# chansoopark98/Deep-Visual-SLAM

Hardware: AMD Instinct MI355X
Metric: VO training-step frames/sec (3-frame 640x480 snippets) (higher is better)
Workload: dtype f32; 1 GPU; configs[2]/[3]: full 4-scale photometric+smoothness loss, batch 12 per GPU, ResNet-18; per_gpu_batch=12, global_batch=12, num_scales=4, image=640x480, parallelism=dp1, streams=depth | pose | 2x weight-gradient, optimizer=fused Adam pass at lr 0: every step computes from the seeded weights, gpu_max_hw_queues=4

## Files before the change

deep-visual-slam_amd/csrc/loss_chain.hip:

```cpp
#include "common.h"

namespace {

constexpr int TW = 64, TH = 16, NT = 256, PX = 4;
constexpr int FH = TH + 2, FW = TW + 2;
constexpr int BH = TH + 4, BW = TW + 4;
constexpr int ACC_W = TW / 2 + 4, ACC_H = TH / 2 + 4;
constexpr int NPART = 16;
constexpr int NDP = 12;
constexpr float C1 = 0.0001f, C2 = 0.0009f;
constexpr float K9 = 1.0f / 9.0f;
#ifndef FWD_WAVES
#define FWD_WAVES 3
#endif
#ifndef BWD_WAVES
#define BWD_WAVES 2
#endif
#ifndef CHAIN_DBG
#define CHAIN_DBG 0
#endif
#ifndef BWD_NT
#define BWD_NT 256
#endif
constexpr int FIELD_ROWS = 6, FIELD_THREADS = FW * (FH / FIELD_ROWS);
static_assert(FH % FIELD_ROWS == 0 && FIELD_THREADS <= NT, "field strips must tile the 1-px-halo tile");
static_assert(ACC_H * ACC_W <= 3 * FH * FW, "sAcc aliases sF");

struct ChainParams {
    dvs_chain_cfg cfg;
    dvs_chain_fwd_io io;
    int tiles_x, tiles_y;
};

struct CamMats {
    float iK[9];
    float P[12];
};

__device__ __forceinline__ float frcp(float x) { return __builtin_amdgcn_rcpf(x); }

__device__ __forceinline__ int reflect_idx(int i, int n) {
    i = i < 0 ? -i : i;
    i = i >= n ? 2 * n - 2 - i : i;
    return min(max(i, 0), n - 1);
}

__device__ __forceinline__ void load_cam(const ChainParams& p, int b, int f, CamMats& m) {
    const float* K = p.io.K + b * 16;
    const float* T = p.io.T[f] + b * 16;
    const float* iK = p.io.inv_K + b * 16;
#pragma unroll
    for (int i = 0; i < 3; ++i) {
#pragma unroll
        for (int j = 0; j < 4; ++j) {
            float acc = K[i * 4 + 0] * T[0 * 4 + j];
            acc = fmaf(K[i * 4 + 1], T[1 * 4 + j], acc);
            acc = fmaf(K[i * 4 + 2], T[2 * 4 + j], acc);
            acc = fmaf(K[i * 4 + 3], T[3 * 4 + j], acc);
            m.P[i * 4 + j] = acc;
        }
#pragma unroll
        for (int j = 0; j < 3; ++j) m.iK[i * 3 + j] = iK[i * 4 + j];
    }
}

__device__ __forceinline__ float disp_up_at(const float* __restrict__ d, int hs, int ws, bool same_res, int W,
                                            int X, int Y, float ry, float rx) {
    if (same_res) return d[Y * W + X];
    float sy = fmaxf(ry * (Y + 0.5f) - 0.5f, 0.f);
    float sx = fmaxf(rx * (X + 0.5f) - 0.5f, 0.f);
    int y0 = min((int)sy, hs - 1), x0 = min((int)sx, ws - 1);
    int y1 = y0 + (y0 < hs - 1), x1 = x0 + (x0 < ws - 1);
    float ly = sy - y0, lx = sx - x0;
    float v00 = d[y0 * ws + x0], v01 = d[y0 * ws + x1];
    float v10 = d[y1 * ws + x0], v11 = d[y1 * ws + x1];
    return (1.f - ly) * ((1.f - lx) * v00 + lx * v01) + ly * ((1.f - lx) * v10 + lx * v11);
}

struct Geo {
    float min_disp, disp_range;
    float inv_wm1, inv_hm1, wm1, hm1;
    int H, W;
};

struct Warp {
    float depth, c0, c1, c2;
    float rden, u, v;
    float gx, gy;
    float mx, my;
    int x0, y0;
    float tx, ty;
    bool in_x1, in_y1;
};

__device__ __forceinline__ void pixel_ray(const float* __restrict__ iK, int X, int Y, float& c0, float& c1, float& c2) {
    float fx = (float)X, fy = (float)Y;
    c0 = fmaf(iK[1], fy, iK[0] * fx) + iK[2];
    c1 = fmaf(iK[4], fy, iK[3] * fx) + iK[5];
    c2 = fmaf(iK[7], fy, iK[6] * fx) + iK[8];
}

__device__ __forceinline__ void warp_project(const float* __restrict__ P, const Geo& g, float depth, float c0, float c1,
                                             float c2, Warp& w) {
    w.depth = depth;
    w.c0 = c0;
    w.c1 = c1;
    w.c2 = c2;
    float X3 = depth * c0, Y3 = depth * c1, Z3 = depth * c2;
    float p0 = fmaf(P[2], Z3, fmaf(P[1], Y3, P[0] * X3)) + P[3];
    float p1 = fmaf(P[6], Z3, fmaf(P[5], Y3, P[4] * X3)) + P[7];
    float p2 = fmaf(P[10], Z3, fmaf(P[9], Y3, P[8] * X3)) + P[11];
    w.rden = frcp(p2 + 1e-7f);
    w.u = p0 * w.rden;
    w.v = p1 * w.rden;
// ... 113 lines not shown
                                            float outb[PX]) {
    float ssa[PX] = {0.f, 0.f, 0.f, 0.f}, ssb[PX] = {0.f, 0.f, 0.f, 0.f};
    float l1a[PX] = {0.f, 0.f, 0.f, 0.f}, l1b[PX] = {0.f, 0.f, 0.f, 0.f};
#pragma unroll 1
    for (int c = 0; c < 3; ++c) {
        const int o = c * PLANE + ly0 * LD + lx;
        const float* xa = sXa + o;
        const float* xb = sXb + o;
        const float* y = sT + o;
        float ry[PX + 2], ryy[PX + 2], ax[PX + 2], axx[PX + 2], axy[PX + 2], bx[PX + 2], bxx[PX + 2], bxy[PX + 2];
#pragma unroll
        for (int j = 0; j < PX + 2; ++j) {
            const float y0 = y[j * LD], y1 = y[j * LD + 1], y2 = y[j * LD + 2];
            const float a0 = xa[j * LD], a1 = xa[j * LD + 1], a2 = xa[j * LD + 2];
            const float b0 = xb[j * LD], b1 = xb[j * LD + 1], b2 = xb[j * LD + 2];
            ry[j] = y0 + y1 + y2;
            ryy[j] = fmaf(y2, y2, fmaf(y1, y1, y0 * y0));
            ax[j] = a0 + a1 + a2;
            axx[j] = fmaf(a2, a2, fmaf(a1, a1, a0 * a0));
            axy[j] = fmaf(a2, y2, fmaf(a1, y1, a0 * y0));
            bx[j] = b0 + b1 + b2;
            bxx[j] = fmaf(b2, b2, fmaf(b1, b1, b0 * b0));
            bxy[j] = fmaf(b2, y2, fmaf(b1, y1, b0 * y0));
            if (j >= 1 && j <= PX) {
                l1a[j - 1] += fabsf(y1 - a1);
                l1b[j - 1] += fabsf(y1 - b1);
            }
        }
#pragma unroll
        for (int k = 0; k < PX; ++k) {
            const float muy = (ry[k] + ry[k + 1] + ry[k + 2]) * K9;
            const float sigy = (ryy[k] + ryy[k + 1] + ryy[k + 2]) * K9 - muy * muy;
            const float my2 = fmaf(muy, muy, C1), sy2 = sigy + C2;
            {
                const float mux = (ax[k] + ax[k + 1] + ax[k + 2]) * K9;
                const float sigx = (axx[k] + axx[k + 1] + axx[k + 2]) * K9 - mux * mux;
                const float sigxy = (axy[k] + axy[k + 1] + axy[k + 2]) * K9 - mux * muy;
                const float n = (2.f * mux * muy + C1) * (2.f * sigxy + C2);
                const float d = fmaf(mux, mux, my2) * (sigx + sy2);
                ssa[k] += fminf(fmaxf((1.f - n * frcp(d)) * 0.5f, 0.f), 1.f);
            }
            {
                const float mux = (bx[k] + bx[k + 1] + bx[k + 2]) * K9;
                const float sigx = (bxx[k] + bxx[k + 1] + bxx[k + 2]) * K9 - mux * mux;
                const float sigxy = (bxy[k] + bxy[k + 1] + bxy[k + 2]) * K9 - mux * muy;
                const float n = (2.f * mux * muy + C1) * (2.f * sigxy + C2);
                const float d = fmaf(mux, mux, my2) * (sigx + sy2);
                ssb[k] += fminf(fmaxf((1.f - n * frcp(d)) * 0.5f, 0.f), 1.f);
            }
        }
    }
#pragma unroll
    for (int k = 0; k < PX; ++k) {
        outa[k] = ssim_ratio * (ssa[k] * (1.f / 3.f)) + (1.f - ssim_ratio) * (l1a[k] * (1.f / 3.f));
        outb[k] = ssim_ratio * (ssb[k] * (1.f / 3.f)) + (1.f - ssim_ratio) * (l1b[k] * (1.f / 3.f));
    }
}

__device__ __forceinline__ void philox4x32(uint32_t c0, uint32_t c1, uint32_t c2, uint32_t c3, uint32_t k0,
                                           uint32_t k1, uint32_t out[4]) {
#pragma unroll
    for (int r = 0; r < 10; ++r) {
        uint32_t hi0 = __umulhi(0xD2511F53u, c0), lo0 = 0xD2511F53u * c0;
        uint32_t hi1 = __umulhi(0xCD9E8D57u, c2), lo1 = 0xCD9E8D57u * c2;
        uint32_t n0 = hi1 ^ c1 ^ k0, n1 = lo1, n2 = hi0 ^ c3 ^ k1, n3 = lo0;
        c0 = n0; c1 = n1; c2 = n2; c3 = n3;
        k0 += 0x9E3779B9u;
        k1 += 0xBB67AE85u;
    }
    out[0] = c0; out[1] = c1; out[2] = c2; out[3] = c3;
}

__device__ __forceinline__ void box_muller(uint32_t a, uint32_t b, float& n0, float& n1) {
    float u1 = ((float)a + 0.5f) * 2.3283064365386963e-10f;
    float u2 = ((float)b + 0.5f) * 2.3283064365386963e-10f;
    float r = sqrtf(-2.f * __logf(u1));
    float s, c;
    __sincosf(6.283185307179586f * u2, &s, &c);
    n0 = r * c;
    n1 = r * s;
}

__device__ __forceinline__ float uni(float v) { return __builtin_bit_cast(float, __builtin_amdgcn_readfirstlane(__builtin_bit_cast(int, v))); }

__device__ __forceinline__ Geo make_geo(const dvs_chain_cfg& c) {
    Geo g;
    g.min_disp = uni(1.0f / c.max_depth);
    g.disp_range = uni(1.0f / c.min_depth - 1.0f / c.max_depth);
    g.wm1 = uni((float)(c.W - 1));
    g.hm1 = uni((float)(c.H - 1));
    g.inv_wm1 = uni(1.0f / g.wm1);
    g.inv_hm1 = uni(1.0f / g.hm1);
    g.H = c.H;
    g.W = c.W;
    return g;
}

template <int PLANE>
__device__ __forceinline__ float edge_weight(const float* __restrict__ sT, int o0, int o1) {
    float gi = fabsf(sT[o0] - sT[o1]) + fabsf(sT[PLANE + o0] - sT[PLANE + o1]) +
               fabsf(sT[2 * PLANE + o0] - sT[2 * PLANE + o1]);
    return __expf(-gi * (1.f / 3.f));
}

constexpr int CAM_STRIDE = 36;
__host__ __device__ __forceinline__ size_t stats_floats(int B, int S) {
    return ((size_t)B * S * 4 + (size_t)B * CAM_STRIDE + 3) / 4 * 4;
}
__device__ __forceinline__ const float* cam_table(const ChainParams& p, int b) {
    return p.io.stats + (size_t)p.cfg.B * p.cfg.num_scales * 4 + (size_t)b * CAM_STRIDE;
}
__device__ __forceinline__ const f4* packed_source(const ChainParams& p, int f, int b) {
    const f4* base = reinterpret_cast<const f4*>(p.io.stats + stats_floats(p.cfg.B, p.cfg.num_scales));
    return base + ((size_t)f * p.cfg.B + b) * ((size_t)p.cfg.H * p.cfg.W);
}

__global__ __launch_bounds__(NT) void chain_pack_kernel(ChainParams p) {
    const int HW = p.cfg.H * p.cfg.W;
    const size_t n = (size_t)2 * p.cfg.B * HW;
    f4* out = reinterpret_cast<f4*>(p.io.stats + stats_floats(p.cfg.B, p.cfg.num_scales));
    for (size_t i = (size_t)blockIdx.x * NT + threadIdx.x; i < n; i += (size_t)gridDim.x * NT) {
        const int pix = (int)(i % HW);
        const size_t fb = i / HW;
        const int b = (int)(fb % p.cfg.B), f = (int)(fb / p.cfg.B);
        const float* src = p.io.source[f] + (size_t)b * 3 * HW + pix;
        out[i] = f4{src[0], src[HW], src[2 * HW], 0.f};
    }
}

__global__ void chain_cam_kernel(ChainParams p) {
    const int b = blockIdx.x, t = threadIdx.x;
    float* out = p.io.stats + (size_t)p.cfg.B * p.cfg.num_scales * 4 + (size_t)b * CAM_STRIDE;
    if (t < 12) {
        const float* iK = p.io.inv_K + b * 16;
        out[t] = (t < 9) ? iK[(t / 3) * 4 + (t % 3)] : 0.f;
    } else if (t < 36) {
        const int f = (t - 12) / 12, e = (t - 12) % 12, i = e / 4, j = e % 4;
        const float* K = p.io.K + b * 16;
        const float* T = p.io.T[f] + b * 16;
        float acc = K[i * 4 + 0] * T[0 * 4 + j];
        acc = fmaf(K[i * 4 + 1], T[1 * 4 + j], acc);
        acc = fmaf(K[i * 4 + 2], T[2 * 4 + j], acc);
        acc = fmaf(K[i * 4 + 3], T[3 * 4 + j], acc);
        out[t] = acc;
    }
}


__global__ __launch_bounds__(NT, FWD_WAVES) void chain_fwd_kernel(ChainParams p) {
    __shared__ float sT[3 * FH * FW];
    __shared__ float sX[2][3 * FH * FW];
    __shared__ float sD[FH * FW];
    __shared__ uint32_t sH[FH * FW];
    __shared__ float sRed[NT / 64][NPART];

    const dvs_chain_cfg& c = p.cfg;
    const int H = c.H, W = c.W, HW = H * W, S = c.num_scales;
    const int b = blockIdx.z, X0 = blockIdx.x * TW, Y0 = blockIdx.y * TH;
    const int tid = threadIdx.x, tx = tid & 63, ty = tid >> 6;
    const Geo geo = make_geo(c);
    constexpr int PL = FH * FW;
    const int X = X0 + tx, Yb = Y0 + PX * ty;

    const float* tgt = p.io.target + (size_t)b * 3 * HW;
    const float* src0 = p.io.source[0] + (size_t)b * 3 * HW;
    const float* src1 = p.io.source[1] + (size_t)b * 3 * HW;
// ... 110 lines not shown
                float i0 = ident[0][k] + n0 * 0.00001f, i1 = ident[1][k] + n1 * 0.00001f;
                best = i0;
                idx = 0;
                if (i1 < best) { best = i1; idx = 1; }
                if (rp[0][k] < best) { best = rp[0][k]; idx = 2; }
            }
            if (rp[1][k] < best) { best = rp[1][k]; idx = 3; }
            a_min += best;
            selbits[k] |= idx << (2 * s);

            int o = (PX * ty + k + 1) * FW + tx + 1;
            float d0 = sD[o];
            a_disp += d0;
            if (X < W - 1) a_gx += fabsf(d0 - sD[o + 1]) * edge_weight<PL>(sT, o, o + 1);
            if (Y < H - 1) a_gy += fabsf(d0 - sD[o + FW]) * edge_weight<PL>(sT, o, o + FW);
        }
        a_min = dvs::wave_sum(a_min);
        a_disp = dvs::wave_sum(a_disp);
        a_gx = dvs::wave_sum(a_gx);
        a_gy = dvs::wave_sum(a_gy);
        if (lane == 0) {
            sRed[wave][s * 4 + 0] = a_min;
            sRed[wave][s * 4 + 1] = a_disp;
            sRed[wave][s * 4 + 2] = a_gx;
            sRed[wave][s * 4 + 3] = a_gy;
        }
        __syncthreads();
    }

#pragma unroll
    for (int k = 0; k < PX; ++k) {
        int Y = Yb + k;
        if (X < W && Y < H) p.io.sel[(size_t)b * HW + (size_t)Y * W + X] = (uint8_t)selbits[k];
    }

    if (tid < NPART) {
        float v = sRed[0][tid] + sRed[1][tid] + sRed[2][tid] + sRed[3][tid];
        int tile = blockIdx.y * p.tiles_x + blockIdx.x;
        p.io.partials[((size_t)b * p.tiles_x * p.tiles_y + tile) * NPART + tid] = v;
    }
}

__global__ __launch_bounds__(NT) void chain_fwd_reduce_kernel(ChainParams p) {
    __shared__ float sRed[NT / 64][NPART];
    const int b = blockIdx.x, ntiles = p.tiles_x * p.tiles_y, tid = threadIdx.x;
    const int col = tid & 15;
    float v = 0.f;
    for (int r = tid >> 4; r < ntiles; r += NT / 16) v += p.io.partials[((size_t)b * ntiles + r) * NPART + col];
    v += __shfl_xor(v, 16, 64);
    v += __shfl_xor(v, 32, 64);
    if ((tid & 63) < 16) sRed[tid >> 6][col] = v;
    __syncthreads();
    if (tid < NPART) {
        float t = sRed[0][tid] + sRed[1][tid] + sRed[2][tid] + sRed[3][tid];
        int s = tid >> 2, j = tid & 3;
        if (s < p.cfg.num_scales) p.io.stats[((size_t)b * p.cfg.num_scales + s) * 4 + j] = t;
    }
}

__global__ void chain_fwd_losses_kernel(ChainParams p) {
    const dvs_chain_cfg& c = p.cfg;
    int s = threadIdx.x;
    if (s >= c.num_scales) return;
    float minsum = 0.f, gx = 0.f, gy = 0.f;
    float hw = (float)c.H * (float)c.W;
    for (int b = 0; b < c.B; ++b) {
        const float* st = p.io.stats + ((size_t)b * c.num_scales + s) * 4;
        float mean = fmaxf(st[1] / hw, 0.001f) + 1e-7f;
        minsum += st[0];
        gx += st[2] / mean;
        gy += st[3] / mean;
    }
    float nx = (float)c.B * (float)c.H * (float)(c.W - 1), ny = (float)c.B * (float)(c.H - 1) * (float)c.W;
    float smooth = gx / nx + gy / ny;
    p.io.losses[s] = minsum / ((float)c.B * hw) + c.smoothness_ratio * smooth / (float)(1 << s);
}

struct BwdParams {
    dvs_chain_bwd_io g;
};

__device__ __forceinline__ float sgn(float v) { return (v > 0.f) ? 1.f : ((v < 0.f) ? -1.f : 0.f); }

template <int NTB, int PXB>
__global__ __launch_bounds__(NTB, NTB == 512 ? 4 : BWD_WAVES) void chain_bwd_kernel(ChainParams p, BwdParams q) {
    static_assert((NTB / 64) * PXB == TH, "waves x rows per lane = tile height");
    constexpr int NWV = NTB / 64;
    constexpr int RING = BH * BW - TH * TW;
    constexpr int FR = NTB == 512 ? 3 : FIELD_ROWS, FT = FW * (FH / FR);
    static_assert(FH % FR == 0 && FT <= NTB, "field strips must tile the 1-px-halo tile");
    __shared__ float sT[3 * BH * BW];
    __shared__ float sX[3 * BH * BW];
    __shared__ float sD[BH * BW];
    __shared__ float sF[3 * FH * FW];
    __shared__ uint8_t sSel[FH * FW];
    __shared__ uint32_t sH[BH * BW];
    __shared__ float sRed[NTB / 64][NDP];
    float* sAcc = sF;

    const dvs_chain_cfg& c = p.cfg;
    const int H = c.H, W = c.W, HW = H * W, S = c.num_scales;
    const int b = blockIdx.z, X0 = blockIdx.x * TW, Y0 = blockIdx.y * TH;
    const int tid0 = threadIdx.x;
    const int wave = tid0 >> 6, lane = tid0 & 63;
    const Geo geo = make_geo(c);
    constexpr int PLB = BH * BW, PLF = FH * FW;
    const int tile = blockIdx.y * p.tiles_x + blockIdx.x, ntiles = p.tiles_x * p.tiles_y;
    int tid = tid0;

    const float* tgt = p.io.target + (size_t)b * 3 * HW;
    for (int i = tid; i < PLB; i += NTB) {
        int hy = i / BW, hx = i - hy * BW;
        int gx = reflect_idx(X0 - 2 + hx, W), gy = reflect_idx(Y0 - 2 + hy, H);
        sH[i] = (uint32_t)gx | ((uint32_t)gy << 16);
#pragma unroll
        for (int ch = 0; ch < 3; ++ch) sT[ch * PLB + i] = tgt[ch * HW + gy * W + gx];
    }
    const float* cam = cam_table(p, b);
    for (int i = tid; i < PLF; i += NTB) {
        int hy = i / FW, hx = i - hy * FW;
        int px = X0 - 1 + hx, py = Y0 - 1 + hy;
        bool in = px >= 0 && px < W && py >= 0 && py < H;
        sSel[i] = in ? p.io.sel[(size_t)b * HW + (size_t)py * W + px] : (uint8_t)0;
    }
    __syncthreads();

    const float w_pix = uni(1.0f / ((float)c.B * (float)HW));
    const float cx = uni(1.0f / ((float)c.B * (float)H * (float)(W - 1)));
    const float cy = uni(1.0f / ((float)c.B * (float)(H - 1) * (float)W));
    const int s_lo = (q.g.scale_end > q.g.scale_begin) ? q.g.scale_begin : 0;
    const int s_hi = (q.g.scale_end > q.g.scale_begin) ? min(q.g.scale_end, S) : S;
#pragma unroll 1
    for (int s = s_lo; s < s_hi; ++s) {
        asm volatile("" : "+v"(tid));
        const int tx = tid & 63, ty = tid >> 6;
        const int X = X0 + tx, Yb = Y0 + PXB * ty;
        const float wxm = (X == 1) ? 2.f : 1.f, wxp = (X == W - 2) ? 2.f : 1.f;
        const int fcol = tid % FW, frow0 = (tid / FW) * FR;
        const bool field_thread = tid < FT;
        const int fpx = X0 - 1 + fcol;
        const int hs = c.hs[s], ws = c.ws[s];
        const bool same_res = (hs == H && ws == W);
        const float* dsp = p.io.disp[s] + (size_t)b * hs * ws;
        const float ry = uni((float)hs / (float)H), rx = uni((float)ws / (float)W);
        const float gl = q.g.d_losses[s];
        const float w_ssim = uni(gl * w_pix * c.ssim_ratio * (1.f / 3.f) * (-0.5f) * K9);
        const float w_l1 = uni(gl * w_pix * (1.f - c.ssim_ratio) * (1.f / 3.f));
        float gd[PXB];
#pragma unroll
        for (int k = 0; k < PXB; ++k) gd[k] = 0.f;

#pragma unroll 1
        for (int f = 0; f < 2; ++f) {
            const float* P = cam + 12 + 12 * f;
            const f4* src4 = packed_source(p, f, b);
            const uint32_t want = 2u + (uint32_t)f;
            auto stage = [&](int i, float (*keep)[2]) __attribute__((always_inline)) {
                const uint32_t h = sH[i];
                const int gx = (int)(h & 0xffffu), gy = (int)(h >> 16);
                float du;
                if (f == 0) {
                    du = disp_up_at(dsp, hs, ws, same_res, W, gx, gy, ry, rx);
                    sD[i] = du;
                } else {
                    du = sD[i];
                }
                float c0, c1, c2;
                pixel_ray(cam, gx, gy, c0, c1, c2);
                Warp w;
                warp_project(P, geo, frcp(geo.min_disp + geo.disp_range * du), c0, c1, c2, w);
                f4 nw, ne, sw, se;
                if (CHAIN_DBG & 1) nw = ne = sw = se = f4{w.u, w.v, w.gx, w.gy};
                else gather_rgba(src4, W, w, nw, ne, sw, se);
                const f4 c4 = bilerp4(w, nw, ne, sw, se);
#pragma unroll
                for (int ch = 0; ch < 3; ++ch) sX[ch * PLB + i] = c4[ch];
                if (keep) {
                    const f4 ddx = ((ne - nw) * (1.f - w.ty) + (se - sw) * w.ty) * (w.mx * w.rden);
                    const f4 ddy = ((sw - nw) * (1.f - w.tx) + (se - ne) * w.tx) * (w.my * w.rden);
#pragma unroll
                    for (int ch = 0; ch < 3; ++ch) {
                        keep[ch][0] = ddx[ch];
                        keep[ch][1] = ddy[ch];
                    }
                }
            };
            float tapd[PXB][3][2];
#pragma unroll
            for (int k = 0; k < PXB; ++k) stage((PXB * ty + k + 2) * BW + tx + 2, tapd[k]);
            for (int j = tid; j < RING; j += NTB) {
                int i;
                if (j < 2 * BW) i = j;
                else if (j < 4 * BW) i = (BH - 4) * BW + j;
                else {
                    const int r = j - 4 * BW, c = r & 3;
                    i = (2 + (r >> 2)) * BW + (c < 2 ? c : BW - 4 + c);
                }
                stage(i, nullptr);
            }
            __syncthreads();

            float dcol[PXB][3];
#pragma unroll 1
            for (int ch = 0; ch < 3; ++ch) {
                if (field_thread && !(CHAIN_DBG & 2)) {
                    const float* xw = sX + ch * PLB + frow0 * BW + fcol;
                    const float* yw = sT + ch * PLB + frow0 * BW + fcol;
                    RowSums r0 = row_sums(xw, yw), r1 = row_sums(xw + BW, yw + BW);
#pragma unroll
                    for (int j = 0; j < FR; ++j) {
                        RowSums r2 = row_sums(xw + (j + 2) * BW, yw + (j + 2) * BW);
                        int hy = frow0 + j, i = hy * FW + fcol, py = Y0 - 1 + hy;
                        float fa = 0.f, fb = 0.f, fc = 0.f;
                        bool in = fpx >= 0 && fpx < W && py >= 0 && py < H;
                        if (in && ((sSel[i] >> (2 * s)) & 3u) == want) {
                            Stats st = stats_of(r0, r1, r2);
                            float n1 = 2.f * st.mux * st.muy + C1, n2 = 2.f * st.sigxy + C2;
                            float d1 = st.mux * st.mux + st.muy * st.muy + C1, d2 = st.sigx + st.sigy + C2;
                            float rd1 = frcp(d1), rd2 = frcp(d2), rd = rd1 * rd2;
                            float R = n1 * n2 * rd, v = (1.f - R) * 0.5f;
                            if (v >= 0.f && v <= 1.f) {
                                float dR_dmux = 2.f * st.muy * n2 * rd - R * 2.f * st.mux * rd1;
                                float dR_dsx = -R * rd2;
                                float dR_dsxy = 2.f * n1 * rd;
                                fa = w_ssim * (dR_dmux - 2.f * st.mux * dR_dsx - st.muy * dR_dsxy);
                                fb = w_ssim * 2.f * dR_dsx;
                                fc = w_ssim * dR_dsxy;
                            }
                        }
                        sF[0 * PLF + i] = fa;
                        sF[1 * PLF + i] = fb;
                        sF[2 * PLF + i] = fc;
                        r0 = r1;
                        r1 = r2;
                    }
                }
                __syncthreads();
                if (CHAIN_DBG & 4) {
#pragma unroll
                    for (int k = 0; k < PXB; ++k) dcol[k][ch] = sX[ch * PLB + (PXB * ty + k + 2) * BW + tx + 2];
                } else {
                    float ha[PXB + 2], hb[PXB + 2], hc[PXB + 2];
#pragma unroll
                    for (int j = 0; j < PXB + 2; ++j) {
                        int o = (PXB * ty + j) * FW + tx;
                        ha[j] = wxm * sF[o] + sF[o + 1] + wxp * sF[o + 2];
                        hb[j] = wxm * sF[PLF + o] + sF[PLF + o + 1] + wxp * sF[PLF + o + 2];
                        hc[j] = wxm * sF[2 * PLF + o] + sF[2 * PLF + o + 1] + wxp * sF[2 * PLF + o + 2];
                    }
#pragma unroll
                    for (int k = 0; k < PXB; ++k) {
                        int Y = Yb + k;
                        float wym = (Y == 1) ? 2.f : 1.f, wyp = (Y == H - 2) ? 2.f : 1.f;
                        float Sa = wym * ha[k] + ha[k + 1] + wyp * ha[k + 2];
                        float Sb = wym * hb[k] + hb[k + 1] + wyp * hb[k + 2];
                        float Sc = wym * hc[k] + hc[k + 1] + wyp * hc[k + 2];
                        int o2 = (PXB * ty + k + 2) * BW + tx + 2;
                        float xq = sX[ch * PLB + o2], yq = sT[ch * PLB + o2];
                        float g = Sa + Sb * xq + Sc * yq;
                        if (((sSel[(PXB * ty + k + 1) * FW + tx + 1] >> (2 * s)) & 3u) == want) g += w_l1 * sgn(xq - yq);
                        dcol[k][ch] = g;
                    }
                }
                __syncthreads();
            }

            float dP[NDP];
#pragma unroll
            for (int j = 0; j < NDP; ++j) dP[j] = 0.f;
#pragma unroll
            for (int k = 0; k < PXB; ++k) {
                int Y = Yb + k;
                if (X >= W || Y >= H) continue;
                if (CHAIN_DBG & 8) {
                    dP[k] += dcol[k][0] + dcol[k][1] + dcol[k][2];
                    continue;
                }
                float du = sD[(PXB * ty + k + 2) * BW + tx + 2];
                float c0, c1, c2;
                pixel_ray(cam, X, Y, c0, c1, c2);
                Warp w;
                warp_project(P, geo, frcp(geo.min_disp + geo.disp_range * du), c0, c1, c2, w);
                float dp0 = 0.f, dp1 = 0.f;
#pragma unroll
                for (int ch = 0; ch < 3; ++ch) {
                    dp0 += dcol[k][ch] * tapd[k][ch][0];
                    dp1 += dcol[k][ch] * tapd[k][ch][1];
                }
                float dp2 = -(dp0 * w.u + dp1 * w.v);
                float X3 = w.depth * w.c0, Y3 = w.depth * w.c1, Z3 = w.depth * w.c2;
                dP[0] += dp0 * X3; dP[1] += dp0 * Y3; dP[2] += dp0 * Z3; dP[3] += dp0;
                dP[4] += dp1 * X3; dP[5] += dp1 * Y3; dP[6] += dp1 * Z3; dP[7] += dp1;
                dP[8] += dp2 * X3; dP[9] += dp2 * Y3; dP[10] += dp2 * Z3; dP[11] += dp2;
                float dc0 = P[0] * dp0 + P[4] * dp1 + P[8] * dp2;
                float dc1 = P[1] * dp0 + P[5] * dp1 + P[9] * dp2;
                float dc2 = P[2] * dp0 + P[6] * dp1 + P[10] * dp2;
                float d_depth = dc0 * w.c0 + dc1 * w.c1 + dc2 * w.c2;
                gd[k] += d_depth * (-w.depth * w.depth * geo.disp_range);
            }
#pragma unroll
            for (int j = 0; j < NDP; ++j) {
                float v = (CHAIN_DBG & 16) ? dP[j] : dvs::wave_sum_lane63(dP[j]);
                if (lane == 63) sRed[wave][j] = v;
            }
            __syncthreads();
            if (tid < NDP) {
                float v = 0.f;
#pragma unroll
                for (int wv = 0; wv < NWV; ++wv) v += sRed[wv][tid];
                q.g.bwd_partials[((((size_t)b * ntiles + tile) * S + s) * 2 + f) * NDP + tid] = v;
            }
            __syncthreads();
        }

        {
            const float* st = p.io.stats + ((size_t)b * S + s) * 4;
            float hw = (float)HW;
            float mean_raw = st[1] / hw;
            float mean = fmaxf(mean_raw, 0.001f) + 1e-7f;
            float gs = gl * c.smoothness_ratio / (float)(1 << s);
            float k_grad = gs / mean;
            float k_mean = (mean_raw >= 0.001f) ? -gs * (cx * st[2] + cy * st[3]) / (mean * mean) / hw : 0.f;
#pragma unroll
            for (int k = 0; k < PXB; ++k) {
                int Y = Yb + k;
                if (X >= W || Y >= H) continue;
                int o = (PXB * ty + k + 2) * BW + tx + 2;
                float d0 = sD[o];
                float g = 0.f;
                if (X < W - 1) g += cx * sgn(d0 - sD[o + 1]) * edge_weight<PLB>(sT, o, o + 1);
                if (X > 0) g -= cx * sgn(sD[o - 1] - d0) * edge_weight<PLB>(sT, o - 1, o);
                if (Y < H - 1) g += cy * sgn(d0 - sD[o + BW]) * edge_weight<PLB>(sT, o, o + BW);
                if (Y > 0) g -= cy * sgn(sD[o - BW] - d0) * edge_weight<PLB>(sT, o - BW, o);
                gd[k] += k_grad * g + k_mean;
            }
        }

        float* dd = q.g.d_disp[s] + (size_t)b * hs * ws;
        if (same_res) {
#pragma unroll
            for (int k = 0; k < PXB; ++k) {
                int Y = Yb + k;
                if (X < W && Y < H) dd[Y * W + X] = gd[k];
            }
        } else {
            for (int i = tid; i < ACC_H * ACC_W; i += NTB) sAcc[i] = 0.f;
            int ox = (int)fmaxf(rx * (X0 + 0.5f) - 0.5f, 0.f), oy = (int)fmaxf(ry * (Y0 + 0.5f) - 0.5f, 0.f);
            __syncthreads();
#pragma unroll
            for (int k = 0; k < PXB; ++k) {
                int Y = Yb + k;
                if (X >= W || Y >= H) continue;
                float sy = fmaxf(ry * (Y + 0.5f) - 0.5f, 0.f), sx = fmaxf(rx * (X + 0.5f) - 0.5f, 0.f);
                int y0 = min((int)sy, hs - 1), x0 = min((int)sx, ws - 1);
                int y1 = y0 + (y0 < hs - 1), x1 = x0 + (x0 < ws - 1);
                float ly = sy - y0, lx = sx - x0;
                float g = gd[k];
                atomicAdd(&sAcc[(y0 - oy) * ACC_W + (x0 - ox)], g * (1.f - ly) * (1.f - lx));
                atomicAdd(&sAcc[(y0 - oy) * ACC_W + (x1 - ox)], g * (1.f - ly) * lx);
                atomicAdd(&sAcc[(y1 - oy) * ACC_W + (x0 - ox)], g * ly * (1.f - lx));
                atomicAdd(&sAcc[(y1 - oy) * ACC_W + (x1 - ox)], g * ly * lx);
            }
            __syncthreads();
            for (int i = tid; i < ACC_H * ACC_W; i += NTB) {
                int ay = i / ACC_W, ax = i - ay * ACC_W;
                float v = sAcc[i];
                int yy = oy + ay, xx = ox + ax;
                if (v != 0.f && yy < hs && xx < ws) atomicAdd(&dd[yy * ws + xx], v);
            }
        }
        __syncthreads();
    }
}

__global__ __launch_bounds__(NT) void chain_bwd_reduce_kernel(ChainParams p, BwdParams q) {
    __shared__ float sRed[NT / 64][16];
    __shared__ float sP[NDP];
    const int b = blockIdx.x, f = blockIdx.y, tid = threadIdx.x;
    const int S = p.cfg.num_scales, ntiles = p.tiles_x * p.tiles_y;
    const int col = tid & 15;
    float v = 0.f;
    if (col < NDP) {
        for (int r = tid >> 4; r < ntiles * S; r += NT / 16) {
            int t = r / S, s = r - t * S;
            v += q.g.bwd_partials[((((size_t)b * ntiles + t) * S + s) * 2 + f) * NDP + col];
        }
    }
    v += __shfl_xor(v, 16, 64);
    v += __shfl_xor(v, 32, 64);
    if ((tid & 63) < 16) sRed[tid >> 6][col] = v;
    __syncthreads();
    if (tid < NDP) sP[tid] = sRed[0][tid] + sRed[1][tid] + sRed[2][tid] + sRed[3][tid];
    __syncthreads();
    if (tid < 16) {
        int k = tid >> 2, j = tid & 3;
        const float* K = p.io.K + b * 16;
        float acc = 0.f;
        for (int i = 0; i < 3; ++i) acc += K[i * 4 + k] * sP[i * 4 + j];
        q.g.d_T[f][b * 16 + tid] = acc;
    }
}

int validate(const dvs_chain_cfg* c, const char* who) {
    DVS_REQUIRE(c, "%s: null cfg", who);
    DVS_REQUIRE(c->B > 0 && c->H >= 4 && c->W >= 4, "%s: bad size B=%d H=%d W=%d", who, c->B, c->H, c->W);
    DVS_REQUIRE(c->num_scales >= 1 && c->num_scales <= DVS_MAX_SCALES, "%s: num_scales=%d", who, c->num_scales);
    for (int s = 0; s < c->num_scales; ++s) {
        DVS_REQUIRE(c->hs[s] > 0 && c->ws[s] > 0, "%s: scale %d is %dx%d", who, s, c->hs[s], c->ws[s]);
        bool same = c->hs[s] == c->H && c->ws[s] == c->W;
        DVS_REQUIRE(same || (c->hs[s] * 2 <= c->H && c->ws[s] * 2 <= c->W),
                    "%s: scale %d (%dx%d) must be full resolution or at most half of %dx%d", who, s, c->hs[s],
                    c->ws[s], c->H, c->W);
    }
    DVS_REQUIRE(c->min_depth > 0.f && c->max_depth > c->min_depth, "%s: depth range", who);
    return DVS_OK;
}

ChainParams make_params(const dvs_chain_cfg* cfg, const dvs_chain_fwd_io* io) {
    ChainParams p;
    p.cfg = *cfg;
    p.io = *io;
    p.tiles_x = (cfg->W + TW - 1) / TW;
    p.tiles_y = (cfg->H + TH - 1) / TH;
    return p;
}

}

extern "C" {

int dvs_chain_workspace(const dvs_chain_cfg* cfg, size_t* partials_bytes, size_t* sel_bytes,
                        size_t* stats_bytes, size_t* bwd_partials_bytes) {
    int rc = validate(cfg, "dvs_chain_workspace");
    if (rc) return rc;
    size_t ntiles = (size_t)((cfg->W + TW - 1) / TW) * ((cfg->H + TH - 1) / TH);
    if (partials_bytes) *partials_bytes = (size_t)cfg->B * ntiles * NPART * sizeof(float);
    if (sel_bytes) *sel_bytes = (size_t)cfg->B * cfg->H * cfg->W;
    if (stats_bytes)
        *stats_bytes = (stats_floats(cfg->B, cfg->num_scales) + (size_t)2 * cfg->B * cfg->H * cfg->W * 4) * sizeof(float);
    if (bwd_partials_bytes) *bwd_partials_bytes = (size_t)cfg->B * ntiles * cfg->num_scales * 2 * NDP * sizeof(float);
    return DVS_OK;
}

int dvs_chain_fwd(const dvs_chain_cfg* cfg, const dvs_chain_fwd_io* io, void* stream) {
    int rc = validate(cfg, "dvs_chain_fwd");
    if (rc) return rc;
    DVS_REQUIRE(io, "dvs_chain_fwd: null io");
    DVS_REQUIRE(io->target && io->source[0] && io->source[1] && io->K && io->inv_K && io->T[0] && io->T[1],
                "dvs_chain_fwd: null input");
    DVS_REQUIRE(io->partials && io->sel && io->stats && io->losses, "dvs_chain_fwd: null workspace/output");
    for (int s = 0; s < cfg->num_scales; ++s) DVS_REQUIRE(io->disp[s], "dvs_chain_fwd: null disp[%d]", s);
    ChainParams p = make_params(cfg, io);
    hipStream_t st = static_cast<hipStream_t>(stream);
    hipLaunchKernelGGL(chain_cam_kernel, dim3(cfg->B), dim3(64), 0, st, p);
    hipLaunchKernelGGL(chain_pack_kernel, dim3(2048), dim3(NT), 0, st, p);
    {
        dvs::ProfScope prof(dvs::SLOT_CHAIN_FWD, st);
        hipLaunchKernelGGL(chain_fwd_kernel, dim3(p.tiles_x, p.tiles_y, cfg->B), dim3(NT), 0, st, p);
    }
    hipLaunchKernelGGL(chain_fwd_reduce_kernel, dim3(cfg->B), dim3(NT), 0, st, p);
    hipLaunchKernelGGL(chain_fwd_losses_kernel, dim3(1), dim3(64), 0, st, p);
    return dvs::check_launch("dvs_chain_fwd");
}

int dvs_chain_bwd(const dvs_chain_cfg* cfg, const dvs_chain_fwd_io* io, const dvs_chain_bwd_io* g,
                  void* stream) {
    int rc = validate(cfg, "dvs_chain_bwd");
    if (rc) return rc;
    DVS_REQUIRE(io && g, "dvs_chain_bwd: null io");
    DVS_REQUIRE(io->target && io->source[0] && io->source[1] && io->K && io->inv_K && io->T[0] && io->T[1],
                "dvs_chain_bwd: null input");
    DVS_REQUIRE(io->sel && io->stats, "dvs_chain_bwd: null forward state");
    DVS_REQUIRE(g->d_losses && g->d_T[0] && g->d_T[1] && g->bwd_partials, "dvs_chain_bwd: null gradient buffer");
    hipStream_t st = static_cast<hipStream_t>(stream);
    DVS_REQUIRE(g->phase >= 0 && g->phase <= 2 && g->scale_begin >= 0 && g->scale_end <= cfg->num_scales, "dvs_chain_bwd: bad phase / scale range");
    const int s_lo = (g->scale_end > g->scale_begin) ? g->scale_begin : 0;
    const int s_hi = (g->scale_end > g->scale_begin) ? g->scale_end : cfg->num_scales;
    for (int s = (g->phase == 2 ? cfg->num_scales : s_lo); s < s_hi; ++s) {
        DVS_REQUIRE(io->disp[s] && g->d_disp[s], "dvs_chain_bwd: null disp/d_disp[%d]", s);
        if (!(cfg->hs[s] == cfg->H && cfg->ws[s] == cfg->W)) {
            hipError_t e = hipMemsetAsync(g->d_disp[s], 0, (size_t)cfg->B * cfg->hs[s] * cfg->ws[s] * sizeof(float), st);
            if (e != hipSuccess) return dvs::fail(DVS_ERR_LAUNCH, "dvs_chain_bwd: memset: %s", hipGetErrorString(e));
        }
    }
    ChainParams p = make_params(cfg, io);
    BwdParams q;
    q.g = *g;
    if (g->phase != 2) {
        dvs::ProfScope prof(dvs::SLOT_CHAIN_BWD, st);
        hipLaunchKernelGGL((chain_bwd_kernel<BWD_NT, TH / (BWD_NT / 64)>), dim3(p.tiles_x, p.tiles_y, cfg->B), dim3(BWD_NT), 0, st, p, q);
    }
    if (g->phase != 1) hipLaunchKernelGGL(chain_bwd_reduce_kernel, dim3(cfg->B, 2), dim3(NT), 0, st, p, q);
    return dvs::check_launch("dvs_chain_bwd");
}

}
```

Measured before the change: 1535 frames/s.

## Compute SSIM backward field in registers with DPP wave shifts and overlapping tiles

The backward chain kernel now uses 62-wide tiles processed by 64 lanes, so each lane computes its own SSIM field values in registers. The horizontal 3-tap sum is done with DPP wave shifts instead of a shared-memory field array. This removes the sF/sSel shared buffers and several __syncthreads per channel, and folds the per-channel dcol accumulation directly into the dp0/dp1 sums. Selection bits are packed into per-lane registers. In exchange there is redundant computation at tile edges, more blocks, more registers per lane, and uniform values are pinned to scalar registers via inline asm.

```diff
diff --git a/deep-visual-slam_amd/csrc/loss_chain.hip b/deep-visual-slam_amd/csrc/loss_chain.hip
--- a/deep-visual-slam_amd/csrc/loss_chain.hip
+++ b/deep-visual-slam_amd/csrc/loss_chain.hip
@@ -4,8 +4,12 @@
 
 constexpr int TW = 64, TH = 16, NT = 256, PX = 4;
 constexpr int FH = TH + 2, FW = TW + 2;
-constexpr int BH = TH + 4, BW = TW + 4;
-constexpr int ACC_W = TW / 2 + 4, ACC_H = TH / 2 + 4;
+#ifndef BWD_PX
+#define BWD_PX 4
+#endif
+constexpr int PXB = BWD_PX, BTW = 62, BTH = (NT / 64) * PXB;
+constexpr int BH = BTH + 4, BW = BTW + 4;
+constexpr int ACC_W = BTW / 2 + 4, ACC_H = BTH / 2 + 4;
 constexpr int NPART = 16;
 constexpr int NDP = 12;
 constexpr float C1 = 0.0001f, C2 = 0.0009f;
@@ -19,17 +23,12 @@
 #ifndef CHAIN_DBG
 #define CHAIN_DBG 0
 #endif
-#ifndef BWD_NT
-#define BWD_NT 256
-#endif
-constexpr int FIELD_ROWS = 6, FIELD_THREADS = FW * (FH / FIELD_ROWS);
-static_assert(FH % FIELD_ROWS == 0 && FIELD_THREADS <= NT, "field strips must tile the 1-px-halo tile");
-static_assert(ACC_H * ACC_W <= 3 * FH * FW, "sAcc aliases sF");
 
 struct ChainParams {
     dvs_chain_cfg cfg;
     dvs_chain_fwd_io io;
     int tiles_x, tiles_y;
+    int btiles_x, btiles_y;
 };
 
 struct CamMats {
@@ -309,6 +308,12 @@
 }
 
 __device__ __forceinline__ float uni(float v) { return __builtin_bit_cast(float, __builtin_amdgcn_readfirstlane(__builtin_bit_cast(int, v))); }
+
+__device__ __forceinline__ float uni_pinned(float v) {
+    float r;
+    asm("v_readfirstlane_b32 %0, %1" : "=s"(r) : "v"(v));
+    return r;
+}
 
 __device__ __forceinline__ Geo make_geo(const dvs_chain_cfg& c) {
     Geo g;
@@ -585,34 +590,35 @@
 
 __device__ __forceinline__ float sgn(float v) { return (v > 0.f) ? 1.f : ((v < 0.f) ? -1.f : 0.f); }
 
-template <int NTB, int PXB>
-__global__ __launch_bounds__(NTB, NTB == 512 ? 4 : BWD_WAVES) void chain_bwd_kernel(ChainParams p, BwdParams q) {
-    static_assert((NTB / 64) * PXB == TH, "waves x rows per lane = tile height");
-    constexpr int NWV = NTB / 64;
-    constexpr int RING = BH * BW - TH * TW;
-    constexpr int FR = NTB == 512 ? 3 : FIELD_ROWS, FT = FW * (FH / FR);
-    static_assert(FH % FR == 0 && FT <= NTB, "field strips must tile the 1-px-halo tile");
+template <int CTRL>
+__device__ __forceinline__ float wave_shift(float v) {
+    return __builtin_bit_cast(float, __builtin_amdgcn_update_dpp(0, __builtin_bit_cast(int, v), CTRL, 0xF, 0xF, true));
+}
+constexpr int DPP_WAVE_SHL1 = 0x130, DPP_WAVE_SHR1 = 0x138;
+
+__global__ __launch_bounds__(NT, BWD_WAVES) void chain_bwd_kernel(ChainParams p, BwdParams q) {
+    constexpr int NWV = NT / 64;
+    constexpr int RING = 4 * BW + 2 * BTH;
+    constexpr int NSEL = (PXB + 2 + 3) / 4;
     __shared__ float sT[3 * BH * BW];
     __shared__ float sX[3 * BH * BW];
     __shared__ float sD[BH * BW];
-    __shared__ float sF[3 * FH * FW];
-    __shared__ uint8_t sSel[FH * FW];
+    __shared__ float sAcc[ACC_H * ACC_W];
     __shared__ uint32_t sH[BH * BW];
-    __shared__ float sRed[NTB / 64][NDP];
-    float* sAcc = sF;
+    __shared__ float sRed[NWV][NDP];
 
     const dvs_chain_cfg& c = p.cfg;
     const int H = c.H, W = c.W, HW = H * W, S = c.num_scales;
-    const int b = blockIdx.z, X0 = blockIdx.x * TW, Y0 = blockIdx.y * TH;
+    const int b = blockIdx.z, X0 = blockIdx.x * BTW, Y0 = blockIdx.y * BTH;
     const int tid0 = threadIdx.x;
     const int wave = tid0 >> 6, lane = tid0 & 63;
     const Geo geo = make_geo(c);
-    constexpr int PLB = BH * BW, PLF = FH * FW;
-    const int tile = blockIdx.y * p.tiles_x + blockIdx.x, ntiles = p.tiles_x * p.tiles_y;
+    constexpr int PLB = BH * BW;
+    const int tile = blockIdx.y * p.btiles_x + blockIdx.x, ntiles = p.btiles_x * p.btiles_y;
     int tid = tid0;
 
     const float* tgt = p.io.target + (size_t)b * 3 * HW;
-    for (int i = tid; i < PLB; i += NTB) {
+    for (int i = tid; i < PLB; i += NT) {
         int hy = i / BW, hx = i - hy * BW;
         int gx = reflect_idx(X0 - 2 + hx, W), gy = reflect_idx(Y0 - 2 + hy, H);
         sH[i] = (uint32_t)gx | ((uint32_t)gy << 16);
@@ -620,38 +626,44 @@
         for (int ch = 0; ch < 3; ++ch) sT[ch * PLB + i] = tgt[ch * HW + gy * W + gx];
     }
     const float* cam = cam_table(p, b);
-    for (int i = tid; i < PLF; i += NTB) {
-        int hy = i / FW, hx = i - hy * FW;
-        int px = X0 - 1 + hx, py = Y0 - 1 + hy;
-        bool in = px >= 0 && px < W && py >= 0 && py < H;
-        sSel[i] = in ? p.io.sel[(size_t)b * HW + (size_t)py * W + px] : (uint8_t)0;
+    uint32_t selp[NSEL];
+#pragma unroll
+    for (int j = 0; j < NSEL; ++j) selp[j] = 0u;
+#pragma unroll
+    for (int j = 0; j < PXB + 2; ++j) {
+        const int px = X0 - 1 + lane, py = Y0 + PXB * wave - 1 + j;
+        const bool in = px >= 0 && px < W && py >= 0 && py < H;
+        const uint32_t v = in ? (uint32_t)p.io.sel[(size_t)b * HW + (size_t)py * W + px] : 0u;
+        selp[j >> 2] |= v << (8 * (j & 3));
     }
     __syncthreads();
 
-    const float w_pix = uni(1.0f / ((float)c.B * (float)HW));
-    const float cx = uni(1.0f / ((float)c.B * (float)H * (float)(W - 1)));
-    const float cy = uni(1.0f / ((float)c.B * (float)(H - 1) * (float)W));
+    const float w_pix = uni_pinned(1.0f / ((float)c.B * (float)HW));
+    const float cx = uni_pinned(1.0f / ((float)c.B * (float)H * (float)(W - 1)));
+    const float cy = uni_pinned(1.0f / ((float)c.B * (float)(H - 1) * (float)W));
+    const float fH = uni_pinned((float)H), fW = uni_pinned((float)W), fHW = uni_pinned((float)HW);
+    const float X0h = uni_pinned(X0 + 0.5f), Y0h = uni_pinned(Y0 + 0.5f);
     const int s_lo = (q.g.scale_end > q.g.scale_begin) ? q.g.scale_begin : 0;
     const int s_hi = (q.g.scale_end > q.g.scale_begin) ? min(q.g.scale_end, S) : S;
 #pragma unroll 1
     for (int s = s_lo; s < s_hi; ++s) {
         asm volatile("" : "+v"(tid));
-        const int tx = tid & 63, ty = tid >> 6;
-        const int X = X0 + tx, Yb = Y0 + PXB * ty;
+        int tx = tid & 63, ty = tid >> 6;
+        int X = X0 - 1 + tx, Yb = Y0 + PXB * ty;
+        bool owner = tx >= 1 && tx <= BTW && X < W;
         const float wxm = (X == 1) ? 2.f : 1.f, wxp = (X == W - 2) ? 2.f : 1.f;
-        const int fcol = tid % FW, frow0 = (tid / FW) * FR;
-        const bool field_thread = tid < FT;
-        const int fpx = X0 - 1 + fcol;
         const int hs = c.hs[s], ws = c.ws[s];
         const bool same_res = (hs == H && ws == W);
         const float* dsp = p.io.disp[s] + (size_t)b * hs * ws;
-        const float ry = uni((float)hs / (float)H), rx = uni((float)ws / (float)W);
-        const float gl = q.g.d_losses[s];
+        const float ry = uni((float)hs / fH), rx = uni((float)ws / fW);
+        const float gl = uni_pinned(q.g.d_losses[s]);
         const float w_ssim = uni(gl * w_pix * c.ssim_ratio * (1.f / 3.f) * (-0.5f) * K9);
         const float w_l1 = uni(gl * w_pix * (1.f - c.ssim_ratio) * (1.f / 3.f));
         float gd[PXB];
 #pragma unroll
         for (int k = 0; k < PXB; ++k) gd[k] = 0.f;
+        if (!same_res)
+            for (int i = tid; i < ACC_H * ACC_W; i += NT) sAcc[i] = 0.f;
 
 #pragma unroll 1
         for (int f = 0; f < 2; ++f) {
@@ -690,82 +702,87 @@
             };
             float tapd[PXB][3][2];
 #pragma unroll
-            for (int k = 0; k < PXB; ++k) stage((PXB * ty + k + 2) * BW + tx + 2, tapd[k]);
-            for (int j = tid; j < RING; j += NTB) {
+            for (int k = 0; k < PXB; ++k) stage((PXB * ty + k + 2) * BW + tx + 1, tapd[k]);
+            for (int j = tid; j < RING; j += NT) {
                 int i;
                 if (j < 2 * BW) i = j;
                 else if (j < 4 * BW) i = (BH - 4) * BW + j;
                 else {
-                    const int r = j - 4 * BW, c = r & 3;
-                    i = (2 + (r >> 2)) * BW + (c < 2 ? c : BW - 4 + c);
+                    const int r = j - 4 * BW;
+                    i = (2 + (r >> 1)) * BW + ((r & 1) ? BW - 1 : 0);
                 }
                 stage(i, nullptr);
             }
             __syncthreads();
 
-            float dcol[PXB][3];
-#pragma unroll 1
+            float dp0s[PXB], dp1s[PXB];
+#pragma unroll
+            for (int k = 0; k < PXB; ++k) dp0s[k] = dp1s[k] = 0.f;
+#pragma unroll
             for (int ch = 0; ch < 3; ++ch) {
-                if (field_thread && !(CHAIN_DBG & 2)) {
-                    const float* xw = sX + ch * PLB + frow0 * BW + fcol;
-                    const float* yw = sT + ch * PLB + frow0 * BW + fcol;
-                    RowSums r0 = row_sums(xw, yw), r1 = row_sums(xw + BW, yw + BW);
-#pragma unroll
-                    for (int j = 0; j < FR; ++j) {
-                        RowSums r2 = row_sums(xw + (j + 2) * BW, yw + (j + 2) * BW);
-                        int hy = frow0 + j, i = hy * FW + fcol, py = Y0 - 1 + hy;
-                        float fa = 0.f, fb = 0.f, fc = 0.f;
-                        bool in = fpx >= 0 && fpx < W && py >= 0 && py < H;
-                        if (in && ((sSel[i] >> (2 * s)) & 3u) == want) {
-                            Stats st = stats_of(r0, r1, r2);
-                            float n1 = 2.f * st.mux * st.muy + C1, n2 = 2.f * st.sigxy + C2;
-                            float d1 = st.mux * st.mux + st.muy * st.muy + C1, d2 = st.sigx + st.sigy + C2;
-                            float rd1 = frcp(d1), rd2 = frcp(d2), rd = rd1 * rd2;
-                            float R = n1 * n2 * rd, v = (1.f - R) * 0.5f;
-                            if (v >= 0.f && v <= 1.f) {
-                                float dR_dmux = 2.f * st.muy * n2 * rd - R * 2.f * st.mux * rd1;
-                                float dR_dsx = -R * rd2;
-                                float dR_dsxy = 2.f * n1 * rd;
-                                fa = w_ssim * (dR_dmux - 2.f * st.mux * dR_dsx - st.muy * dR_dsxy);
-                                fb = w_ssim * 2.f * dR_dsx;
-                                fc = w_ssim * dR_dsxy;
-                            }
-                        }
-                        sF[0 * PLF + i] = fa;
-                        sF[1 * PLF + i] = fb;
-                        sF[2 * PLF + i] = fc;
-                        r0 = r1;
-                        r1 = r2;
+                const float* xw = sX + ch * PLB + PXB * ty * BW + tx;
+                const float* yw = sT + ch * PLB + PXB * ty * BW + tx;
+                RowSums rs[PXB + 4];
+                float xq[PXB], yq[PXB];
+#pragma unroll
+                for (int r = 0; r < PXB + 4; ++r) {
+                    const float x0 = xw[r * BW], x1 = xw[r * BW + 1], x2 = xw[r * BW + 2];
+                    const float y0 = yw[r * BW], y1 = yw[r * BW + 1], y2 = yw[r * BW + 2];
+                    rs[r].x = x0 + x1 + x2;
+                    rs[r].y = y0 + y1 + y2;
+                    rs[r].xx = fmaf(x2, x2, fmaf(x1, x1, x0 * x0));
+                    rs[r].yy = fmaf(y2, y2, fmaf(y1, y1, y0 * y0));
+                    rs[r].xy = fmaf(x2, y2, fmaf(x1, y1, x0 * y0));
+                    if (r >= 2 && r < PXB + 2) {
+                        xq[r - 2] = x1;
+                        yq[r - 2] = y1;
                     }
                 }
-                __syncthreads();
-                if (CHAIN_DBG & 4) {
-#pragma unroll
-                    for (int k = 0; k < PXB; ++k) dcol[k][ch] = sX[ch * PLB + (PXB * ty + k + 2) * BW + tx + 2];
-                } else {
-                    float ha[PXB + 2], hb[PXB + 2], hc[PXB + 2];
-#pragma unroll
-                    for (int j = 0; j < PXB + 2; ++j) {
-                        int o = (PXB * ty + j) * FW + tx;
-                        ha[j] = wxm * sF[o] + sF[o + 1] + wxp * sF[o + 2];
-                        hb[j] = wxm * sF[PLF + o] + sF[PLF + o + 1] + wxp * sF[PLF + o + 2];
-                        hc[j] = wxm * sF[2 * PLF + o] + sF[2 * PLF + o + 1] + wxp * sF[2 * PLF + o + 2];
+                float ha[PXB + 2], hb[PXB + 2], hc[PXB + 2];
+#pragma unroll
+                for (int j = 0; j < PXB + 2; ++j) {
+                    float fa, fb, fc;
+                    if (CHAIN_DBG & 2) {
+                        fa = rs[j].x; fb = rs[j + 1].y; fc = rs[j + 2].xy;
+                    } else {
+                        const bool on = ((selp[j >> 2] >> (8 * (j & 3) + 2 * s)) & 3u) == want;
+                        const Stats st = stats_of(rs[j], rs[j + 1], rs[j + 2]);
+                        const float n1 = 2.f * st.mux * st.muy + C1, n2 = 2.f * st.sigxy + C2;
+                        const float d1 = st.mux * st.mux + st.muy * st.muy + C1, d2 = st.sigx + st.sigy + C2;
+                        const float rd1 = frcp(d1), rd2 = frcp(d2), rd = rd1 * rd2;
+                        const float R = n1 * n2 * rd, v = (1.f - R) * 0.5f;
+                        const float dR_dmux = 2.f * st.muy * n2 * rd - R * 2.f * st.mux * rd1;
+                        const float dR_dsx = -R * rd2;
+                        const float dR_dsxy = 2.f * n1 * rd;
+                        const bool live = on && v >= 0.f && v <= 1.f;
+                        fa = live ? w_ssim * (dR_dmux - 2.f * st.mux * dR_dsx - st.muy * dR_dsxy) : 0.f;
+                        fb = live ? w_ssim * 2.f * dR_dsx : 0.f;
+                        fc = live ? w_ssim * dR_dsxy : 0.f;
                     }
-#pragma unroll
-                    for (int k = 0; k < PXB; ++k) {
-                        int Y = Yb + k;
-                        float wym = (Y == 1) ? 2.f : 1.f, wyp = (Y == H - 2) ? 2.f : 1.f;
-                        float Sa = wym * ha[k] + ha[k + 1] + wyp * ha[k + 2];
-                        float Sb = wym * hb[k] + hb[k + 1] + wyp * hb[k + 2];
-                        float Sc = wym * hc[k] + hc[k + 1] + wyp * hc[k + 2];
-                        int o2 = (PXB * ty + k + 2) * BW + tx + 2;
-                        float xq = sX[ch * PLB + o2], yq = sT[ch * PLB + o2];
-                        float g = Sa + Sb * xq + Sc * yq;
-                        if (((sSel[(PXB * ty + k + 1) * FW + tx + 1] >> (2 * s)) & 3u) == want) g += w_l1 * sgn(xq - yq);
-                        dcol[k][ch] = g;
+                    if (CHAIN_DBG & 4) {
+                        ha[j] = wxm * fa + fa + wxp * fa;
+                        hb[j] = wxm * fb + fb + wxp * fb;
+                        hc[j] = wxm * fc + fc + wxp * fc;
+                    } else {
+                        ha[j] = wxm * wave_shift<DPP_WAVE_SHR1>(fa) + fa + wxp * wave_shift<DPP_WAVE_SHL1>(fa);
+                        hb[j] = wxm * wave_shift<DPP_WAVE_SHR1>(fb) + fb + wxp * wave_shift<DPP_WAVE_SHL1>(fb);
+                        hc[j] = wxm * wave_shift<DPP_WAVE_SHR1>(fc) + fc + wxp * wave_shift<DPP_WAVE_SHL1>(fc);
                     }
                 }
-                __syncthreads();
+#pragma unroll
+                for (int k = 0; k < PXB; ++k) {
+                    const int Y = Yb + k;
+                    const float wym = (Y == 1) ? 2.f : 1.f, wyp = (Y == H - 2) ? 2.f : 1.f;
+                    const float Sa = wym * ha[k] + ha[k + 1] + wyp * ha[k + 2];
+                    const float Sb = wym * hb[k] + hb[k + 1] + wyp * hb[k + 2];
+                    const float Sc = wym * hc[k] + hc[k + 1] + wyp * hc[k + 2];
+                    const float g = Sa + Sb * xq[k] + Sc * yq[k];
+                    const bool mine = ((selp[(k + 1) >> 2] >> (8 * ((k + 1) & 3) + 2 * s)) & 3u) == want;
+                    const float dcol = g + (mine ? w_l1 * sgn(xq[k] - yq[k]) : 0.f);
+                    dp0s[k] += dcol * tapd[k][ch][0];
+                    dp1s[k] += dcol * tapd[k][ch][1];
+                    asm volatile("" : "+v"(dp0s[k]), "+v"(dp1s[k]));
+                }
             }
 
             float dP[NDP];
@@ -774,22 +791,17 @@
 #pragma unroll
             for (int k = 0; k < PXB; ++k) {
                 int Y = Yb + k;
-                if (X >= W || Y >= H) continue;
+                if (!owner || Y >= H) continue;
                 if (CHAIN_DBG & 8) {
-                    dP[k] += dcol[k][0] + dcol[k][1] + dcol[k][2];
+                    dP[k] += dp0s[k] + dp1s[k];
                     continue;
                 }
-                float du = sD[(PXB * ty + k + 2) * BW + tx + 2];
+                float du = sD[(PXB * ty + k + 2) * BW + tx + 1];
                 float c0, c1, c2;
                 pixel_ray(cam, X, Y, c0, c1, c2);
                 Warp w;
                 warp_project(P, geo, frcp(geo.min_disp + geo.disp_range * du), c0, c1, c2, w);
-                float dp0 = 0.f, dp1 = 0.f;
-#pragma unroll
-                for (int ch = 0; ch < 3; ++ch) {
-                    dp0 += dcol[k][ch] * tapd[k][ch][0];
-                    dp1 += dcol[k][ch] * tapd[k][ch][1];
-                }
+                const float dp0 = dp0s[k], dp1 = dp1s[k];
                 float dp2 = -(dp0 * w.u + dp1 * w.v);
                 float X3 = w.depth * w.c0, Y3 = w.depth * w.c1, Z3 = w.depth * w.c2;
                 dP[0] += dp0 * X3; dP[1] += dp0 * Y3; dP[2] += dp0 * Z3; dP[3] += dp0;
@@ -813,22 +825,26 @@
                 for (int wv = 0; wv < NWV; ++wv) v += sRed[wv][tid];
                 q.g.bwd_partials[((((size_t)b * ntiles + tile) * S + s) * 2 + f) * NDP + tid] = v;
             }
-            __syncthreads();
-        }
+        }
+
+        asm volatile("" : "+v"(tid));
+        tx = tid & 63, ty = tid >> 6;
+        X = X0 - 1 + tx, Yb = Y0 + PXB * ty;
+        owner = tx >= 1 && tx <= BTW && X < W;
 
         {
             const float* st = p.io.stats + ((size_t)b * S + s) * 4;
-            float hw = (float)HW;
+            float hw = fHW;
             float mean_raw = st[1] / hw;
             float mean = fmaxf(mean_raw, 0.001f) + 1e-7f;
             float gs = gl * c.smoothness_ratio / (float)(1 << s);
-            float k_grad = gs / mean;
-            float k_mean = (mean_raw >= 0.001f) ? -gs * (cx * st[2] + cy * st[3]) / (mean * mean) / hw : 0.f;
+            float k_grad = uni(gs / mean);
+            float k_mean = uni((mean_raw >= 0.001f) ? -gs * (cx * st[2] + cy * st[3]) / (mean * mean) / hw : 0.f);
 #pragma unroll
             for (int k = 0; k < PXB; ++k) {
                 int Y = Yb + k;
-                if (X >= W || Y >= H) continue;
-                int o = (PXB * ty + k + 2) * BW + tx + 2;
+                if (!owner || Y >= H) continue;
+                int o = (PXB * ty + k + 2) * BW + tx + 1;
                 float d0 = sD[o];
                 float g = 0.f;
                 if (X < W - 1) g += cx * sgn(d0 - sD[o + 1]) * edge_weight<PLB>(sT, o, o + 1);
@@ -844,16 +860,14 @@
 #pragma unroll
             for (int k = 0; k < PXB; ++k) {
                 int Y = Yb + k;
-                if (X < W && Y < H) dd[Y * W + X] = gd[k];
+                if (owner && Y < H) dd[Y * W + X] = gd[k];
             }
         } else {
-            for (int i = tid; i < ACC_H * ACC_W; i += NTB) sAcc[i] = 0.f;
-            int ox = (int)fmaxf(rx * (X0 + 0.5f) - 0.5f, 0.f), oy = (int)fmaxf(ry * (Y0 + 0.5f) - 0.5f, 0.f);
-            __syncthreads();
+            int ox = (int)fmaxf(rx * X0h - 0.5f, 0.f), oy = (int)fmaxf(ry * Y0h - 0.5f, 0.f);
 #pragma unroll
             for (int k = 0; k < PXB; ++k) {
                 int Y = Yb + k;
-                if (X >= W || Y >= H) continue;
+                if (!owner || Y >= H) continue;
                 float sy = fmaxf(ry * (Y + 0.5f) - 0.5f, 0.f), sx = fmaxf(rx * (X + 0.5f) - 0.5f, 0.f);
                 int y0 = min((int)sy, hs - 1), x0 = min((int)sx, ws - 1);
                 int y1 = y0 + (y0 < hs - 1), x1 = x0 + (x0 < ws - 1);
@@ -865,7 +879,7 @@
                 atomicAdd(&sAcc[(y1 - oy) * ACC_W + (x1 - ox)], g * ly * lx);
             }
             __syncthreads();
-            for (int i = tid; i < ACC_H * ACC_W; i += NTB) {
+            for (int i = tid; i < ACC_H * ACC_W; i += NT) {
                 int ay = i / ACC_W, ax = i - ay * ACC_W;
                 float v = sAcc[i];
                 int yy = oy + ay, xx = ox + ax;
@@ -880,7 +894,7 @@
     __shared__ float sRed[NT / 64][16];
     __shared__ float sP[NDP];
     const int b = blockIdx.x, f = blockIdx.y, tid = threadIdx.x;
-    const int S = p.cfg.num_scales, ntiles = p.tiles_x * p.tiles_y;
+    const int S = p.cfg.num_scales, ntiles = p.btiles_x * p.btiles_y;
     const int col = tid & 15;
     float v = 0.f;
     if (col < NDP) {
@@ -925,6 +939,8 @@
     p.io = *io;
     p.tiles_x = (cfg->W + TW - 1) / TW;
     p.tiles_y = (cfg->H + TH - 1) / TH;
+    p.btiles_x = (cfg->W + BTW - 1) / BTW;
+    p.btiles_y = (cfg->H + BTH - 1) / BTH;
     return p;
 }
 
@@ -941,7 +957,8 @@
     if (sel_bytes) *sel_bytes = (size_t)cfg->B * cfg->H * cfg->W;
     if (stats_bytes)
         *stats_bytes = (stats_floats(cfg->B, cfg->num_scales) + (size_t)2 * cfg->B * cfg->H * cfg->W * 4) * sizeof(float);
-    if (bwd_partials_bytes) *bwd_partials_bytes = (size_t)cfg->B * ntiles * cfg->num_scales * 2 * NDP * sizeof(float);
+    size_t bntiles = (size_t)((cfg->W + BTW - 1) / BTW) * ((cfg->H + BTH - 1) / BTH);
+    if (bwd_partials_bytes) *bwd_partials_bytes = (size_t)cfg->B * bntiles * cfg->num_scales * 2 * NDP * sizeof(float);
     return DVS_OK;
 }
 
@@ -991,7 +1008,7 @@
     q.g = *g;
     if (g->phase != 2) {
         dvs::ProfScope prof(dvs::SLOT_CHAIN_BWD, st);
-        hipLaunchKernelGGL((chain_bwd_kernel<BWD_NT, TH / (BWD_NT / 64)>), dim3(p.tiles_x, p.tiles_y, cfg->B), dim3(BWD_NT), 0, st, p, q);
+        hipLaunchKernelGGL(chain_bwd_kernel, dim3(p.btiles_x, p.btiles_y, cfg->B), dim3(NT), 0, st, p, q);
     }
     if (g->phase != 1) hipLaunchKernelGGL(chain_bwd_reduce_kernel, dim3(cfg->B, 2), dim3(NT), 0, st, p, q);
     return dvs::check_launch("dvs_chain_bwd");
```

After: 1543 frames/s, median of 6. About the same (+0.5%).
